# nanoporetech/isONclust2

Measured on AMD Instinct MI355X. Metric: reads/s clustered (sahlin mode, k=11 w=15), higher is better.
Workload: dtype u32

## Files before the change

### isonclust2_amd/csrc/ioc_align_gpu.hip

```cpp
#include <hip/hip_runtime.h>

#include <algorithm>
#include <chrono>
#include <cmath>
#include <cstdint>
#include <cstring>
#include <numeric>
#include <string>
#include <type_traits>
#include <vector>

#include "ioc_align_sink.h"
#include "ioc_internal.h"

namespace {

constexpr int ALN_C = 8;
constexpr int ALN_MAXW = 8;
constexpr int ALN_NEG = INT32_MIN / 4;
constexpr uint32_t ALN_LEN_SHIFT = 26;

struct AlnPairDev {
    uint32_t q_off, n;
    uint32_t r_off, m;
// ... 1539 lines not shown
    uint32_t* split;
    size_t resume_words;
};

int v2_tables(ioc_ctx* c, const V2Plan& pl, uint32_t help_wgs, V2Dev& t)
{
    hipStream_t s = c->stream;
    const uint32_t ncouples = pl.ncouples, np = pl.np;
    const size_t tab_bytes = size_t(ncouples) * sizeof(V2Couple) + size_t(np) * (sizeof(V2PairCk) + sizeof(V2PairEnd)) + size_t(pl.max_items) * sizeof(V2Item) + 256;
    IOC_TRY(ioc_reserve(c, c->a_cko, tab_bytes));
    uint8_t* tb = static_cast<uint8_t*>(c->a_cko.p);
    t.cps = reinterpret_cast<V2Couple*>(tb);
    t.pck = reinterpret_cast<V2PairCk*>(tb + size_t(ncouples) * sizeof(V2Couple));
    t.pend = reinterpret_cast<V2PairEnd*>(reinterpret_cast<uint8_t*>(t.pck) + size_t(np) * sizeof(V2PairCk));
    t.items = reinterpret_cast<V2Item*>(reinterpret_cast<uint8_t*>(t.pend) + size_t(np) * sizeof(V2PairEnd));
    IOC_CHK(c, hipMemcpyAsync(t.cps, pl.cps.data(), size_t(ncouples) * sizeof(V2Couple), hipMemcpyHostToDevice, s));
    IOC_CHK(c, hipMemcpyAsync(t.pck, pl.pck.data(), size_t(np) * sizeof(V2PairCk), hipMemcpyHostToDevice, s));
    IOC_CHK(c, hipMemcpyAsync(t.pend, pl.pend.data(), size_t(np) * sizeof(V2PairEnd), hipMemcpyHostToDevice, s));
    IOC_TRY(ioc_reserve(c, c->a_prof, size_t(pl.prof_total) * sizeof(uint4) + 256));
    IOC_TRY(ioc_reserve(c, c->a_ends2, size_t(np) * sizeof(int4)));
    IOC_TRY(ioc_reserve(c, c->a_lrow, (size_t(pl.lrow_total) + pl.best_total + 16) * sizeof(int2)));
    t.lrow = static_cast<int2*>(c->a_lrow.p);
    t.best = t.lrow + pl.lrow_total;
    t.ctl_words = ((16 + 2 * size_t(pl.max_flags) + np + 1) & ~size_t(1)) + 2;
    IOC_TRY(ioc_reserve(c, c->a_xflags, t.ctl_words * 4));
    t.ctl = static_cast<uint32_t*>(c->a_xflags.p);
    const size_t n_scratch = size_t(pl.max_pairs) + size_t(help_wgs) * V2_NHELP * V2_HBUF;
    t.resume_words = size_t(np) * V2_RESUME_WORDS + 2u * (size_t(pl.max_pairs) + 1u) + 4u + size_t(np) * V2_SPLIT_WORDS;
    IOC_TRY(ioc_reserve(c, c->a_bnd, n_scratch * sizeof(V2Scratch) + t.resume_words * 4));
    t.scratch = static_cast<V2Scratch*>(c->a_bnd.p);
    t.hscratch = t.scratch + pl.max_pairs;
    t.resume = reinterpret_cast<uint32_t*>(t.scratch + n_scratch);
    t.park = t.resume + size_t(np) * V2_RESUME_WORDS;
    t.early = t.park + size_t(pl.max_pairs) + 1u;
    t.gate = t.early + size_t(pl.max_pairs) + 1u;
    t.split = t.gate + 4u;
    return IOC_OK;
}

uint32_t v2_per_cu(const V2Plan& pl, size_t si, const V2Opts& o, bool few_couples)
{
    if (few_couples) return uint32_t(o.occ);
    uint64_t tiles = 0;
    uint32_t diags = 1;
    for (uint32_t k2 = pl.slices[si].first; k2 < pl.slices[si].first + pl.slices[si].second; ++k2) {
        const V2Couple& cp = pl.cps[k2];
        for (uint32_t b = 0; b < cp.nbands; ++b) tiles += uint32_t(cp.phi[b]) - uint32_t(cp.plo[b]) + 1u;
        diags = std::max(diags, cp.nbands + cp.nstrips - 1u);
    }
    const double x = double(tiles) / double(diags) / double(uint32_t(o.n_cu) * uint32_t(V2_WAVES));
    return x < 1.0 ? 1u : x < 2.75 ? std::min(2u, uint32_t(o.occ)) : uint32_t(o.occ);
}

int v2_slice(ioc_ctx* c, const V2Plan& pl, const V2Dev& t, size_t si, const V2Opts& o, const AlnParams& P, const uint32_t* d_order,
             int32_t* d_score, uint32_t* d_count, const hipEvent_t* ev, uint32_t* xe, const AlnOpsDev* od, StageTrace& tr)
{
    hipStream_t s = c->stream;
    const uint32_t k_first = pl.slices[si].first, n_couples = pl.slices[si].second;
    const uint32_t first_pair = 2u * k_first, n_pairs = std::min(pl.cnt, 2u * (k_first + n_couples)) - first_pair;
    const uint32_t n_items = pl.n_items[si], n_probe = pl.n_probe[si];
    const AlnPairDev* d_pairs = static_cast<const AlnPairDev*>(c->a_pairs.p);
    const uint8_t* d_pool = static_cast<const uint8_t*>(c->a_pool.p);
    uint32_t* d_ctl = t.ctl;
    const bool few_couples = n_couples <= o.few_limit;
    const uint32_t prog_every = few_couples ? 1u : 0u;
    const bool items_check = !pl.items.empty();
    if (items_check)
        IOC_CHK(c, hipMemsetAsync(t.items, 0xFF, size_t(n_items) * sizeof(V2Item), s));
    hipLaunchKernelGGL(k_fwd2_items, dim3(pl.n_diag[si], 2), dim3(V2_ITEMS_T), 0, s, t.cps, k_first, n_couples, n_probe, t.items, n_items);
    IOC_CHK(c, hipGetLastError());
    if (items_check) IOC_TRY(device_items_check(c, pl, t.items, si));
    hipLaunchKernelGGL(k_fwd2_prof, dim3(n_couples, pl.max_strips), dim3(128), 0, s, d_pairs, t.cps + k_first, d_pool, P, static_cast<uint4*>(c->a_prof.p));
    IOC_CHK(c, hipGetLastError());
    IOC_CHK(c, hipMemsetAsync(d_ctl, 0, t.ctl_words * 4, s));
    IOC_CHK(c, hipMemsetAsync(t.resume, 0, t.resume_words * 4, s));
    if (pl.tiles_skipped)
        IOC_CHK(c, hipMemsetAsync(t.lrow, 0x80, (size_t(pl.lrow_total) + pl.best_total) * sizeof(int2), s));
    if (getenv("IOC_ALIGN_V2_FAKE_TIMEOUT")) {
        const uint32_t one = 1;
        IOC_CHK(c, hipMemcpyAsync(d_ctl + 1, &one, 4, hipMemcpyHostToDevice, s));
    }
    IOC_CHK(c, hipEventRecord(ev[0], s));
    auto fwd = [&](decltype(&k_fwd2) kernel, uint32_t n_wg, const V2Item* items, uint32_t n) {
        hipLaunchKernelGGL(kernel, dim3(n_wg), dim3(64 * V2_WAVES), 0, s, d_pairs, t.cps, items, n, d_ctl, d_ctl + 16, d_ctl + 1, d_pool, P,
                           static_cast<uint32_t*>(c->a_ck.p), t.lrow, t.best, d_ctl + 16 + 2 * pl.max_flags, o.guard, static_cast<const uint4*>(c->a_prof.p),
                           reinterpret_cast<unsigned long long*>(d_ctl + t.ctl_words - 2), few_couples ? d_ctl + 16 + pl.max_flags : static_cast<uint32_t*>(nullptr),
                           prog_every);
    };
    if (n_probe) {
        fwd(k_fwd2, std::max(1u, std::min(uint32_t(o.occ) * uint32_t(o.n_cu), (n_probe + V2_WAVES - 1) / V2_WAVES)), t.items, n_probe);
        IOC_CHK(c, hipGetLastError());
        hipLaunchKernelGGL(k_fwd2_probe, dim3(n_couples), dim3(64), 0, s, d_pairs, t.cps + k_first, t.pend, static_cast<const uint32_t*>(c->a_ck.p), P);
        IOC_CHK(c, hipGetLastError());
        IOC_CHK(c, hipMemsetAsync(d_ctl, 0, 4, s));
    }
    tr.mark("v2_slice up to the probe");
    const uint32_t n_main = n_items - n_probe, per_cu = v2_per_cu(pl, si, o, few_couples);
    const uint32_t n_wg = std::max(1u, std::min(per_cu * uint32_t(o.n_cu), (n_main + V2_WAVES - 1) / V2_WAVES));
    const bool w2 = per_cu <= 2 && !getenv("IOC_ALIGN_V2_NO_W2");
    if (getenv("IOC_TRACE"))
        fprintf(stderr, "[ioc]   aligner v2: shape: slice %zu: %u couples, waits for %s, per_cu %u, n_wg %u, kernel %s, n_probe %u\n", si, n_couples,
                few_couples ? "rows" : "tiles", per_cu, n_wg, w2 ? "k_fwd2_w2" : "k_fwd2", n_probe);
    fwd(w2 ? k_fwd2_w2 : k_fwd2, n_wg, t.items + n_probe, n_main);
    IOC_CHK(c, hipGetLastError());
    const uint32_t n_help = std::min<uint32_t>(n_pairs, o.help_wgs);
    hipLaunchKernelGGL(k_fwd2_ends, dim3(n_pairs), dim3(64), 0, s, d_pairs, t.cps, d_order + first_pair, n_pairs, t.pend, t.lrow, t.best,
                       d_ctl + 16 + 2 * pl.max_flags, static_cast<int4*>(c->a_ends2.p), t.resume, t.early, o.side_help ? int(P.match) : 0, n_help);
    IOC_CHK(c, hipGetLastError());
    IOC_CHK(c, hipEventRecord(ev[1], s));
    auto help = [&](hipStream_t hs, uint32_t* list, uint32_t which, uint32_t* gate) {
        if (od)
            hipLaunchKernelGGL(k_trace2_help_ops, dim3(n_help), dim3(64 * V2_HWAVES), 0, hs, d_pairs, d_order + first_pair, d_pool, P,
                               static_cast<const uint32_t*>(c->a_ck.p), t.cps, t.pck, static_cast<const int4*>(c->a_ends2.p), t.scratch, t.hscratch,
                               t.resume, list, t.split, d_score, d_count, n_pairs, which, gate, *od);
        else
            hipLaunchKernelGGL(k_trace2_help, dim3(n_help), dim3(64 * V2_HWAVES), 0, hs, d_pairs, d_order + first_pair, d_pool, P,
                               static_cast<const uint32_t*>(c->a_ck.p), t.cps, t.pck, static_cast<const int4*>(c->a_ends2.p), t.scratch, t.hscratch,
                               t.resume, list, t.split, d_score, d_count, n_pairs, which, gate);
    };
    if (o.side_help) {
        IOC_CHK(c, hipEventRecord(c->ev_side[0], s));
        IOC_CHK(c, hipStreamWaitEvent(c->side_stream, c->ev_side[0], 0));
        help(c->side_stream, t.early, 2u, t.gate);
        IOC_CHK(c, hipGetLastError());
        IOC_CHK(c, hipEventRecord(c->ev_side[1], c->side_stream));
        hipLaunchKernelGGL(k_trace2_gate, dim3(1), dim3(1), 0, s, t.early, t.gate, n_help);
        IOC_CHK(c, hipGetLastError());
    }
    if (od)
        hipLaunchKernelGGL(k_trace2_ops, dim3((n_pairs + TR_WAVES - 1) / TR_WAVES), dim3(64 * TR_WAVES), 0, s, d_pairs, d_order + first_pair, d_pool, P,
                           static_cast<const uint32_t*>(c->a_ck.p), t.cps, t.pck, static_cast<const int4*>(c->a_ends2.p), t.scratch, t.resume, t.park,
                           t.split, d_score, d_count, n_pairs, o.deadline, o.deadline_cycles, *od);
    else
        hipLaunchKernelGGL(k_trace2, dim3((n_pairs + TR_WAVES - 1) / TR_WAVES), dim3(64 * TR_WAVES), 0, s, d_pairs, d_order + first_pair, d_pool, P,
                           static_cast<const uint32_t*>(c->a_ck.p), t.cps, t.pck, static_cast<const int4*>(c->a_ends2.p), t.scratch, t.resume, t.park,
                           t.split, d_score, d_count, n_pairs, o.deadline, o.deadline_cycles);
    IOC_CHK(c, hipGetLastError());
    if (o.side_help) IOC_CHK(c, hipStreamWaitEvent(s, c->ev_side[1], 0));
    if (o.deadline) {
        help(s, t.park, 1u, nullptr);
        IOC_CHK(c, hipGetLastError());
    }
    IOC_CHK(c, hipEventRecord(ev[2], s));
    unsigned long long cells_done = 0;
    IOC_CHK(c, hipMemcpyAsync(xe, d_ctl + 1, 4, hipMemcpyDeviceToHost, s));
    IOC_CHK(c, hipMemcpyAsync(&cells_done, d_ctl + t.ctl_words - 2, 8, hipMemcpyDeviceToHost, s));
    tr.mark("v2_slice other launches");
    IOC_CHK(c, hipStreamSynchronize(s));
    tr.mark("v2_slice wait (device)");
    c->tm.n_align_cells_computed += int64_t(cells_done);
    if (items_check) IOC_TRY(device_probe_report(c, pl, t.cps, si));
    return IOC_OK;
}

int v2_report(ioc_ctx* c, const std::vector<AlnPairDev>& dp, const uint32_t* order, const V2Plan& pl, const V2Dev& t, size_t si, uint32_t deadline)
{
    const bool rates = getenv("IOC_V2_TRACE_RATES") != nullptr, times = getenv("IOC_V2_TRACE_TIMES") != nullptr;
    if (!rates && !times) return IOC_OK;
    const uint32_t np = pl.np, first_pair = 2u * pl.slices[si].first;
    const uint32_t n_pairs = std::min(pl.cnt, 2u * (pl.slices[si].first + pl.slices[si].second)) - first_pair;
    std::vector<int4> he(np);
    IOC_CHK(c, hipMemcpy(he.data(), c->a_ends2.p, size_t(np) * sizeof(int4), hipMemcpyDeviceToHost));
    if (rates)
        for (uint32_t x = 0; x < n_pairs; ++x) {
            const uint32_t pid = order[first_pair + x];
            const AlnPairDev& d = dp[pid];
            fprintf(stderr, "[rate] e %.5f n %u m %u score %d per_base %.5f go %d flags %d corridor %u\n", double(d.e_sum), d.n, d.m, he[pid].x,
                    double(he[pid].x) / double(std::max(d.n, d.m)), d.gap_open, he[pid].w, pl.cps[pl.pend[pid].couple].corridor);
        }
    if (!times) return IOC_OK;
    std::vector<uint32_t> rw(size_t(np) * V2_RESUME_WORDS);
    IOC_CHK(c, hipMemcpy(rw.data(), t.resume, rw.size() * 4, hipMemcpyDeviceToHost));
    std::vector<uint32_t> ids(n_pairs);
// ... 139 lines not shown
    tr.mark("tile_counts");

    o.deadline = 4;
    if (const char* e = getenv("IOC_TRACE2_DEADLINE")) o.deadline = uint32_t(std::max(0, atoi(e)));
    if (const char* e = getenv("IOC_TRACE2_CYCLES")) o.deadline_cycles = (unsigned long long)std::max(0.0, atof(e));
    o.help_wgs = o.deadline ? std::min<uint32_t>(pl.max_pairs, uint32_t(o.n_cu)) : 0u;
    V2Dev t{};
    if ((r = v2_tables(c, pl, o.help_wgs, t)) != IOC_OK) return r;
    tr.mark("v2_tables");
    o.side_help = o.deadline && !(getenv("IOC_TRACE2_EARLY") && atoi(getenv("IOC_TRACE2_EARLY")) == 0);
    if (o.side_help && !c->side_stream) {
        IOC_CHK(c, hipStreamCreateWithFlags(&c->side_stream, hipStreamNonBlocking));
        for (auto& e : c->ev_side) IOC_CHK(c, hipEventCreateWithFlags(&e, hipEventDisableTiming));
    }
    EventSet evs;
    evs.v.assign(pl.slices.size() * 3, nullptr);
    for (auto& e : evs.v) IOC_CHK(c, hipEventCreate(&e));
    tr.mark("side stream, events");
    if (getenv("IOC_TRACE"))
        fprintf(stderr, "[ioc]   aligner v2: planning (couples, corridors, tile lists, tables) took the host %.3f ms\n",
                std::chrono::duration<double, std::milli>(std::chrono::steady_clock::now() - t_plan0).count());
    size_t evi = 0;
    bool bad = false;
    for (size_t si = 0; si < pl.slices.size() && !bad; ++si, evi += 3) {
        uint32_t xe = 0;
        if ((r = v2_slice(c, pl, t, si, o, P, d_order, d_score, d_count, &evs.v[evi], &xe, ops ? &ops->dev : nullptr, tr)) != IOC_OK) return r;
        if (ops && !xe) {
            const uint32_t x0 = 2u * pl.slices[si].first, x1 = std::min(cnt, 2u * (pl.slices[si].first + pl.slices[si].second));
            if ((r = ops_fetch(c, *ops, dp, order + x0, d_order + x0, x1 - x0, slice_ops[si])) != IOC_OK) return r;
        }
        if ((r = v2_report(c, dp, order, pl, t, si, o.deadline)) != IOC_OK) return r;
        bad = xe != 0;
    }
    add_elapsed(c, evs.v, evi);
    tr.mark("elapsed times");
    if (getenv("IOC_TRACE"))
        fprintf(stderr, "[ioc]   aligner v2: forward %.3f ms, traceback %.3f ms (device, all slices so far)%s\n", c->tm.ms_align_fwd,
                c->tm.ms_align_trace, bad ? " — a wait ran out: falling back to version 1" : "");
    *fell_back = bad;
    return IOC_OK;
}


enum class AlnRoute { normal, every_tile, v1_only };

struct AlnOut {
    int32_t* score;
    int64_t* windows;
    double* ratio;
    const AlnSink* ops = nullptr;
    void set(size_t i, int32_t s, int64_t w, double r) const
    {
        if (score) score[i] = s;
        if (windows) windows[i] = w;
        if (ratio) ratio[i] = r;
    }
};

// ... 620 lines not shown
```

### isonclust2_amd/csrc/ioc_align_v2.inc

```

constexpr int CK2 = 512;
constexpr int V2_WAVES = 4;
constexpr int V2_BLK_C = 8;
constexpr int V2_MAX_BANDS = 40;
static_assert(CK2 % TILE == 0 && CK2 == 64 * V2_BLK_C, "block geometry");

struct V2Couple {
    uint32_t pid[2];
    uint32_t nbands, nstrips;
    uint32_t tpb;
    uint32_t flag0;
    uint32_t mpad;
    uint32_t nq;
    uint64_t rdat;
    uint64_t rbase;
    uint64_t cdat;
    uint64_t cbase;
    uint64_t prof;
    uint32_t lrow0[2];
    uint32_t best0[2];
    uint16_t bstart[V2_MAX_BANDS + 1];
    uint16_t plo[V2_MAX_BANDS], phi[V2_MAX_BANDS];
    uint32_t corridor;
    uint16_t probe_band, probe_strip;
// ... 88 lines not shown
        e = umax2(e, h);
        h = umax2(T[c], e) - gd2;
        Hq[c] = h;
    }
    hql = h;
    el = e;
}

__device__ __forceinline__ uint32_t v2_par(uint32_t lds_byte_addr)
{
    uint32_t x;
    asm volatile("ds_read_b32 %0, %1\n\ts_waitcnt lgkmcnt(0)" : "=v"(x) : "v"(lds_byte_addr) : "memory");
    return x;
}

__device__ __forceinline__ void v2_lds_store(uint32_t lds_byte_addr, uint32_t v)
{
    asm volatile("ds_write_b32 %0, %1\n\ts_waitcnt lgkmcnt(0)" : : "v"(lds_byte_addr), "v"(v) : "memory");
}

enum V2Par : uint32_t {
    VP_N0 = 0, VP_N1, VP_M0, VP_M1, VP_GD0, VP_GD1, VP_LROW0, VP_LROW1, VP_BEST0, VP_BEST1, VP_PID0, VP_PID1,
    VP_RDAT_LO, VP_RDAT_HI, VP_RBASE_LO, VP_RBASE_HI, VP_CDAT_LO, VP_CDAT_HI, VP_CBASE_LO, VP_CBASE_HI,
    VP_MPAD, VP_NQ, VP_FLAG, VP_BAND, VP_STRIP, VP_COLIN_LO, VP_COLIN_HI, VP_RHI0, VP_RHI1, VP_COUNT = 32
};

__global__ void __launch_bounds__(128)
k_fwd2_prof(const AlnPairDev* __restrict__ pairs, const V2Couple* __restrict__ couples, const uint8_t* __restrict__ pool, AlnParams P, uint4* __restrict__ prof)
{
    const V2Couple& cp = couples[blockIdx.x];
    const uint32_t p = blockIdx.y;
    if (p >= cp.nstrips) return;
    const uint32_t h = threadIdx.x >> 6, lane = threadIdx.x & 63u;
    const bool have = cp.pid[h] != 0xFFFFFFFFu;
    const AlnPairDev pr = pairs[have ? cp.pid[h] : cp.pid[0]];
    const uint32_t m = have ? pr.m : 0u;
    const uint8_t* r = pool + pr.r_off;
    const int ge = P.gap_extend, gd = pr.gap_open - ge;
    const int cm = P.match + 2 * ge + gd, cx = P.mismatch + 2 * ge + gd;
    const uint32_t jb = p * (64u * FW_C) + lane * FW_C;
    uint32_t rpk[FW_C / 4];
#pragma unroll
    for (int c4 = 0; c4 < FW_C / 4; ++c4) {
        uint32_t w = 0;
#pragma unroll
        for (int e = 0; e < 4; ++e) w |= (have ? ref_byte(r, m, pr.rc, jb + c4 * 4 + e) : 0u) << (8 * e);
        rpk[c4] = w;
// ... 57 lines not shown
                cnt = min(dg, nb - 1u) - b_lo + 1u;
            }
        }
        s_scan[tid] = cnt;
        __syncthreads();
        for (uint32_t d = 1; d < V2_ITEMS_T; d <<= 1) {
            const uint32_t v = tid >= d ? s_scan[tid - d] : 0u;
            __syncthreads();
            s_scan[tid] += v;
            __syncthreads();
        }
        const uint32_t pos = running + s_scan[tid] - cnt;
        for (uint32_t i = 0; i < cnt; ++i)
            if (pos + i < n_items) items[pos + i] = V2Item{k_first + x, uint16_t(b_lo + i), uint16_t(dg - (b_lo + i))};
        running += s_scan[V2_ITEMS_T - 1];
        __syncthreads();
    }
}

static __device__ __forceinline__ void
v2_fwd_body(const AlnPairDev* __restrict__ pairs, const V2Couple* __restrict__ couples, const V2Item* __restrict__ items, uint32_t n_items,
       uint32_t* __restrict__ queue, uint32_t* __restrict__ flags, uint32_t* __restrict__ err, const uint8_t* __restrict__ pool, AlnParams P,
       uint32_t* __restrict__ arena, int2* __restrict__ lrow, int2* __restrict__ bandbest, uint32_t* __restrict__ ovf_out, int guard,
       const uint4* __restrict__ prof, unsigned long long* __restrict__ cells_done, uint32_t* __restrict__ prog, uint32_t prog_every)
{
    __shared__ __attribute__((aligned(16))) uint32_t s_look_all[V2_WAVES][3][128];
    __shared__ __attribute__((aligned(16))) uint32_t s_prof_all[V2_WAVES][2][5][64][4];
    __shared__ uint32_t s_par_all[V2_WAVES][VP_COUNT];
    const uint32_t lane = threadIdx.x & 63u;
    const uint32_t wv = uint32_t(__builtin_amdgcn_readfirstlane(int(threadIdx.x >> 6)));
    uint32_t(*s_look)[128] = s_look_all[wv];
    uint32_t* s_par = s_par_all[wv];
    const uint32_t par_addr = uint32_t(reinterpret_cast<uintptr_t>(s_par));
    auto par = [&](uint32_t k) -> uint32_t { return v2_par(par_addr + 4u * k); };
    auto par64 = [&](uint32_t k) -> uint64_t { return uint64_t(par(k)) | (uint64_t(par(k + 1u)) << 32); };
    constexpr uint32_t strip_cols = 64u * FW_C;
    const int ge = P.gap_extend;
    auto qcode = [](uint32_t ch) -> uint32_t {
        const uint32_t code = ch == 'A' ? 0u : ch == 'C' ? 1u : ch == 'G' ? 2u : ch == 'T' ? 3u : 4u;
        return code * 1024u;
    };
    uint32_t it = v2_dequeue(queue);
    while (it < n_items) {
        uint32_t band, p, r_lo, nblk[2];
        bool vh[2], last_band[2];
        bool left_ok = true;
        bool top_none = false;
        bool left_rows = false;
        uint32_t left_idx = 0, nblk_band = 0, left_avail = 0;
        const uint8_t* q[2];
        int base[2];
        uint32_t gd2;
        uint32_t Hp[FW_C], F[FW_C];
        uint32_t dg;
        uint64_t cb_off = 0;
        uint64_t co_off = 0;
        uint64_t rd_off = 0;
        uint64_t rb_off = 0;
        uint32_t mpad = 0, ncr = 0;
        {
            const V2Item item = items[it];
            const V2Couple cp = couples[item.couple];
            band = item.band;
            p = item.strip;
            if (p < cp.plo[band] || p > cp.phi[band] ||
                __builtin_amdgcn_readfirstlane(int(__hip_atomic_load(&flags[cp.flag0 + band * cp.nstrips + p], __ATOMIC_RELAXED, __HIP_MEMORY_SCOPE_AGENT))) != 0) {
                it = v2_dequeue(queue);
                continue;
            }
            const bool top_in = band > 0 && p >= cp.plo[band - 1u] && p <= cp.phi[band - 1u];
            const bool left_in = p > cp.plo[band];
            left_ok = p == 0 || left_in;
            top_none = band > 0 && !top_in;
            const bool corner_in = band > 0 && p > 0 && p - 1u >= cp.plo[band - 1u] && p - 1u <= cp.phi[band - 1u];
            if (top_in) (void)v2_wait(&flags[cp.flag0 + (band - 1u) * cp.nstrips + p], err);
            left_rows = prog != nullptr && left_in;
            left_idx = cp.flag0 + band * cp.nstrips + (p - 1u);
            {
                const uint32_t rows_b = min(max(cp.pid[0] != 0xFFFFFFFFu ? pairs[cp.pid[0]].n : 0u, cp.pid[1] != 0xFFFFFFFFu ? pairs[cp.pid[1]].n : 0u),
                                            uint32_t(cp.bstart[band + 1u]) * uint32_t(CK2));
                const uint32_t r0_b = uint32_t(cp.bstart[band]) * uint32_t(CK2);
                nblk_band = rows_b > r0_b ? (rows_b - r0_b + FW_R - 1) / FW_R : 0u;
            }
            if (left_in && !left_rows) (void)v2_wait(&flags[left_idx], err);
            if (left_rows) (void)v2_wait_rows(&prog[left_idx], &flags[left_idx], min(32u, nblk_band), err, left_avail);
            __builtin_amdgcn_fence(__ATOMIC_ACQUIRE, "agent");
            r_lo = uint32_t(cp.bstart[band]) * uint32_t(CK2);
            const uint32_t jb = p * strip_cols + lane * FW_C;
            uint32_t n[2], m[2], r_hi[2];
            int gd[2];
#pragma unroll
            for (int h = 0; h < 2; ++h) {
                const bool have = cp.pid[h] != 0xFFFFFFFFu;
                const AlnPairDev pr = pairs[have ? cp.pid[h] : cp.pid[0]];
                n[h] = have ? pr.n : 0u;
                m[h] = have ? pr.m : 0u;
                q[h] = pool + pr.q_off;
                gd[h] = pr.gap_open - ge;
                r_hi[h] = min(n[h], uint32_t(cp.bstart[band + 1u]) * uint32_t(CK2));
                nblk[h] = r_hi[h] > r_lo ? (r_hi[h] - r_lo + FW_R - 1) / FW_R : 0u;
                const uint32_t nstr = (m[h] + strip_cols - 1) / strip_cols;
                vh[h] = have && p < nstr && nblk[h] > 0;
                last_band[h] = vh[h] && r_hi[h] == n[h];
            }
            gd2 = packu(uint32_t(gd[0]), uint32_t(gd[1]));
            mpad = cp.mpad;
            rd_off = cp.rdat + jb;
            rb_off = cp.rbase + uint64_t(jb / 16u) * 2u;
            {
                uint32_t nmx = max(n[0], n[1]);
                ncr = nmx ? (nmx - 1u) / uint32_t(CK2) : 0u;
            }
            {
                const uint64_t e0 = uint64_t((jb + FW_C) / CK2 - ((jb + FW_C) >= uint32_t(CK2) ? 1u : 0u)) * cp.nq + r_lo / 4u;
                co_off = cp.cdat + e0 * 8u;
                cb_off = cp.cbase + e0 * 2u;
            }
            const uint64_t colin = p ? uint64_t(p * (strip_cols / CK2) - 1u) * cp.nq : 0;
            __builtin_amdgcn_fence(__ATOMIC_RELEASE, "workgroup");
            __builtin_amdgcn_wave_barrier();
            if (lane == 0) {
                s_par[VP_N0] = n[0];
                s_par[VP_N1] = n[1];
                s_par[VP_M0] = m[0];
                s_par[VP_M1] = m[1];
                s_par[VP_GD0] = uint32_t(gd[0]);
                s_par[VP_GD1] = uint32_t(gd[1]);
                s_par[VP_LROW0] = cp.lrow0[0];
                s_par[VP_LROW1] = cp.lrow0[1];
                s_par[VP_BEST0] = cp.best0[0];
                s_par[VP_BEST1] = cp.best0[1];
                s_par[VP_PID0] = cp.pid[0];
                s_par[VP_PID1] = cp.pid[1];
                s_par[VP_RDAT_LO] = uint32_t(cp.rdat);
                s_par[VP_RDAT_HI] = uint32_t(cp.rdat >> 32);
                s_par[VP_RBASE_LO] = uint32_t(cp.rbase);
                s_par[VP_RBASE_HI] = uint32_t(cp.rbase >> 32);
                s_par[VP_CDAT_LO] = uint32_t(cp.cdat);
                s_par[VP_CDAT_HI] = uint32_t(cp.cdat >> 32);
                s_par[VP_CBASE_LO] = uint32_t(cp.cbase);
                s_par[VP_CBASE_HI] = uint32_t(cp.cbase >> 32);
                s_par[VP_MPAD] = cp.mpad;
                s_par[VP_NQ] = cp.nq;
                s_par[VP_FLAG] = cp.flag0 + band * cp.nstrips + p;
                s_par[VP_BAND] = band;
                s_par[VP_STRIP] = p;
                s_par[VP_COLIN_LO] = uint32_t(colin);
                s_par[VP_COLIN_HI] = uint32_t(colin >> 32);
                s_par[VP_RHI0] = r_hi[0];
                s_par[VP_RHI1] = r_hi[1];
            }
            int Ha[2][FW_C], Fa[2][FW_C], dga[2];
#pragma unroll
            for (int h = 0; h < 2; ++h) {
                if (!vh[h]) {
#pragma unroll
                    for (int c = 0; c < FW_C; ++c) Ha[h][c] = Fa[h][c] = 0;
                    dga[h] = 0;
                } else if (r_lo > 0 && !top_in) {
#pragma unroll
                    for (int c = 0; c < FW_C; ++c) Ha[h][c] = Fa[h][c] = ALN_NEG;
                    dga[h] = ALN_NEG;
                } else if (r_lo == 0) {
                    const int b0 = ge * int(jb) - gd[h];
#pragma unroll
                    for (int c = 0; c < FW_C; ++c) {
                        Ha[h][c] = b0 + ge * (c + 1);
                        Fa[h][c] = ALN_NEG;
                    }
                    dga[h] = b0;
                } else {
                    const uint32_t ckr = r_lo / CK2 - 1u;
                    const uint32_t* rh = arena + cp.rdat + uint64_t(2u * ckr) * cp.mpad;
// ... 24 lines not shown
                    base[h] = v2_half(d[0], h) + (h ? bb.y : bb.x) - U16_BIAS;
                } else
                base[h] = __builtin_amdgcn_readfirstlane(Ha[h][0]) - U16_BIAS;
            }
#pragma unroll
            for (int c = 0; c < FW_C; ++c) {
                const bool in0 = vh[0] && jb + c < m[0], in1 = vh[1] && jb + c < m[1];
                Hp[c] = packu(in0 ? clampu16(Ha[0][c] - base[0]) : uint32_t(U16_BIAS), in1 ? clampu16(Ha[1][c] - base[1]) : uint32_t(U16_BIAS));
                F[c] = packu(in0 ? clampu16(Fa[0][c] - base[0]) : uint32_t(U16_BIAS), in1 ? clampu16(Fa[1][c] - base[1]) : uint32_t(U16_BIAS));
            }
            dg = packu(clampu16(dga[0] - base[0]), clampu16(dga[1] - base[1]));
            {
                const uint4* pp = prof + cp.prof + uint64_t(p) * (2u * 5u * 64u) + lane;
#pragma unroll
                for (int h = 0; h < 2; ++h)
#pragma unroll
                    for (int code = 0; code < 5; ++code) {
                        const uint4 w = pp[(uint32_t(h) * 5u + uint32_t(code)) * 64u];
                        *reinterpret_cast<uint4*>(&s_prof_all[wv][h][code][lane][0]) = w;
                    }
            }
        }
        const uint32_t jb = p * strip_cols + lane * FW_C;
        const uint32_t nsteps = max(nblk[0], nblk[1]) + 63u;
        uint32_t lanef = 0;
        int lastc[2];
        uint32_t ncl[2];
        bool strip_has_lastc = false;
        __builtin_amdgcn_fence(__ATOMIC_RELEASE, "workgroup");
        __builtin_amdgcn_wave_barrier();
        __builtin_amdgcn_fence(__ATOMIC_ACQUIRE, "workgroup");
        {
            const uint32_t jr = jb + FW_C;
            bool any_right = false;
#pragma unroll
            for (int h = 0; h < 2; ++h) {
                const uint32_t mh = par(VP_M0 + h);
                const bool hc = vh[h] && jb < mh;
                ncl[h] = vh[h] ? min(64u, (mh - p * strip_cols + FW_C - 1) / FW_C) : 0u;
                lastc[h] = (vh[h] && mh - 1 >= jb && mh - 1 < jb + FW_C) ? int(mh - 1 - jb) : -1;
                strip_has_lastc = strip_has_lastc || (vh[h] && uint64_t(p + 1u) * strip_cols >= mh);
                any_right = any_right || (vh[h] && jr < mh);
                lanef |= (hc ? 1u : 0u) << h;
                lanef |= (lastc[h] >= 0 ? 4u : 0u) << h;
            }
            if ((jr % CK2) == 0 && any_right) lanef |= 16u;
        }
// ... 35 lines not shown
                en[h] = left_edge(h, row);
            }
            qn = qq[0] | (qq[1] << 16);
        };
        fetch(0);
        publish(0);
        fetch(1);
        __builtin_amdgcn_fence(__ATOMIC_RELEASE, "workgroup");
        __builtin_amdgcn_wave_barrier();
        __builtin_amdgcn_fence(__ATOMIC_ACQUIRE, "workgroup");
        uint4 nxh, nxe, nxq;
        nxh = *reinterpret_cast<const uint4*>(&s_look[0][0]);
        nxe = *reinterpret_cast<const uint4*>(&s_look[1][0]);
        nxq = *reinterpret_cast<const uint4*>(&s_look[2][0]);
        {
            const uint32_t q4[FW_R] = {nxq.x, nxq.y, nxq.z, nxq.w};
#pragma unroll
            for (int rr = 0; rr < FW_R; ++rr) qc[rr] = from_left_or(qc[rr], q4[rr]);
        }
        int bc[2] = {ALN_NEG, ALN_NEG};
        uint32_t bc_i[2] = {0, 0};
        uint32_t ovf = 0;

        auto step = [&](const uint32_t s, auto first) __attribute__((always_inline)) {
            if (decltype(first)::value && (s & (64 / FW_R - 1)) == 0) {
                if (s) {
                    int dl[2];
#pragma unroll
                    for (int h = 0; h < 2; ++h) {
                        const uint32_t lr = s + 1u > nblk[h] ? min(63u, s + 1u - nblk[h]) : 0u;
                        const int ref = __builtin_amdgcn_readlane(int(Hp[0]), int(lr));
                        dl[h] = max(v2_half(uint32_t(ref), h) - U16_BIAS, 0);
                        if (!vh[h] || lr >= ncl[h]) dl[h] = 0;
                        base[h] += dl[h];
                    }
                    const uint32_t d2 = packu(uint32_t(dl[0]), uint32_t(dl[1]));
                    {
                        uint32_t mx = Hp[0], mn = Hp[0];
#pragma unroll
                        for (int c = 1; c < FW_C; ++c) {
                            mx = umax2(mx, Hp[c]);
                            mn = umin2(mn, Hp[c]);
                        }
                        const int bi = int(s) - int(lane);
#pragma unroll
                        for (int h = 0; h < 2; ++h) {
                            const int hi_v = v2_half(mx, h) - U16_BIAS, lo_v = v2_half(mn, h) - U16_BIAS;
                            if ((lanef >> h & 1u) && bi >= (top_none ? 1 : 0) && uint32_t(bi) < nblk[h] && (hi_v > guard || lo_v < -guard)) {
// ... 6 lines not shown
                    }
#pragma unroll
                    for (int c = 0; c < FW_C; ++c) {
                        Hp[c] = usubs2(Hp[c], d2);
                        F[c] = usubs2(F[c], d2);
                    }
                    dg = usubs2(dg, d2);
#pragma unroll
                    for (int rr = 0; rr < FW_R; ++rr) {
                        hl[rr] = usubs2(hl[rr], d2);
                        el[rr] = usubs2(el[rr], d2);
                    }
                    nxh = uint4{usubs2(nxh.x, d2), usubs2(nxh.y, d2), usubs2(nxh.z, d2), usubs2(nxh.w, d2)};
                    nxe = uint4{usubs2(nxe.x, d2), usubs2(nxe.y, d2), usubs2(nxe.z, d2), usubs2(nxe.w, d2)};
                    const uint32_t cur = ((s / (64 / FW_R)) & 1u) * 64u + lane;
                    s_look[0][cur] = usubs2(s_look[0][cur], d2);
                    s_look[1][cur] = usubs2(s_look[1][cur], d2);
                }
                const uint32_t blk = s / (64 / FW_R) + 1u;
                if (prog != nullptr && s >= 64u && (prog_every <= 1u || (s / 16u) % prog_every == 0u)) {
                    asm volatile("s_waitcnt vmcnt(0)" ::: "memory");
                    __builtin_amdgcn_fence(__ATOMIC_RELEASE, "agent");
                    asm volatile("s_waitcnt vmcnt(0)" ::: "memory");
                    __hip_atomic_store(&prog[uint32_t(__builtin_amdgcn_readfirstlane(int(par(VP_FLAG))))], s - 63u, __ATOMIC_RELAXED, __HIP_MEMORY_SCOPE_AGENT);
                }
                publish(blk);
                if (left_rows) {
                    const uint32_t need_rows = min(16u * (blk + 2u), nblk_band);
                    if (need_rows > left_avail) {
                        (void)v2_wait_rows(&prog[left_idx], &flags[left_idx], need_rows, err, left_avail);
                        __builtin_amdgcn_fence(__ATOMIC_ACQUIRE, "agent");
                    }
                }
                fetch(blk + 1u);
            }
            {
                const uint32_t h4[FW_R] = {nxh.x, nxh.y, nxh.z, nxh.w}, e4[FW_R] = {nxe.x, nxe.y, nxe.z, nxe.w};
#pragma unroll
                for (int rr = 0; rr < FW_R; ++rr) {
                    hl[rr] = from_left_or(hl[rr], h4[rr]);
                    el[rr] = from_left_or(el[rr], e4[rr]);
                }
                const uint32_t nx = ((s + 1u) * FW_R) & 127u;
                nxh = *reinterpret_cast<const uint4*>(&s_look[0][nx]);
                nxe = *reinterpret_cast<const uint4*>(&s_look[1][nx]);
                nxq = *reinterpret_cast<const uint4*>(&s_look[2][nx]);
            }
// ... 1 lines not shown
            bool act[2];
#pragma unroll
            for (int h = 0; h < 2; ++h) act[h] = (lanef >> h & 1u) && bi >= 0 && uint32_t(bi) < nblk[h];
            if (act[0] || act[1]) {
                const bool special = strip_has_lastc || (last_band[0] && s + 1u >= nblk[0] && s + 1u - nblk[0] < 64u) ||
                                     (last_band[1] && s + 1u >= nblk[1] && s + 1u - nblk[1] < 64u);
                auto row_cells = [&](int rr) __attribute__((always_inline)) {
                    const uint32_t hl_in = hl[rr];
                    const uint4 xa = *reinterpret_cast<const uint4*>(profA + (qc[rr] & 0xFFFFu));
                    const uint4 xb = *reinterpret_cast<const uint4*>(profB + (qc[rr] >> 16));
                    cells_u16(Hp, F, xa, xb, hl[rr], el[rr], dg, gd2);
                    dg = hl_in;
                };
#pragma unroll
                for (int rr = 0; rr < FW_R; ++rr) {
                    row_cells(rr);
                    if (special) {

#pragma unroll
                        for (int h = 0; h < 2; ++h) {
                            const uint32_t i = r_lo + uint32_t(bi) * FW_R + rr;
                            const uint32_t nh = par(VP_N0 + h), mh = par(VP_M0 + h);
                            const int gdh = int(par(VP_GD0 + h));
                            if (act[h] && i < nh) {
                                if (lastc[h] >= 0) {
                                    const uint32_t lc = uint32_t(lastc[h]);
                                    const bool b0 = lc & 1u, b1 = lc & 2u, b2 = lc & 4u, b3 = lc & 8u;
                                    const uint32_t s0 = b0 ? Hp[1] : Hp[0], s1 = b0 ? Hp[3] : Hp[2], s2 = b0 ? Hp[5] : Hp[4], s3 = b0 ? Hp[7] : Hp[6],
                                                   s4 = b0 ? Hp[9] : Hp[8], s5 = b0 ? Hp[11] : Hp[10], s6 = b0 ? Hp[13] : Hp[12], s7 = b0 ? Hp[15] : Hp[14];
                                    const uint32_t u0 = b1 ? s1 : s0, u1 = b1 ? s3 : s2, u2 = b1 ? s5 : s4, u3 = b1 ? s7 : s6;
                                    const uint32_t v0 = b2 ? u1 : u0, v1 = b2 ? u3 : u2;
                                    int hm = v2_half(b3 ? v1 : v0, h) + base[h];
                                    hm += gdh - ge * int(i + 1u + mh);
                                    if (hm > bc[h]) {
                                        bc[h] = hm;
                                        bc_i[h] = i + 1u;
                                    }
                                }
                                if (i + 1u == nh) {
                                    int br = ALN_NEG;
                                    uint32_t bj = 0;
                                    const int b0 = base[h] + gdh - ge * int(nh + jb);
#pragma unroll
                                    for (int c = 0; c < FW_C; ++c) {
                                        const int ht = v2_half(Hp[c], h) + b0 - ge * (c + 1);
                                        if (jb + c < mh && ht > br) {
// ... 25 lines not shown
#pragma unroll
                        for (int c = 0; c < FW_C; c += 4) {
                            oh[c / 4] = uint4{Hp[c], Hp[c + 1], Hp[c + 2], Hp[c + 3]};
                            of[c / 4] = uint4{F[c], F[c + 1], F[c + 2], F[c + 3]};
                        }
                        reinterpret_cast<int2*>(arena + rb_off)[uint64_t(ckr1 - 1u) * (mpad / 16u)] = int2{base[0], base[1]};
                    }
                }
            }
            {
                const uint32_t q4[FW_R] = {nxq.x, nxq.y, nxq.z, nxq.w};
#pragma unroll
                for (int rr = 0; rr < FW_R; ++rr) qc[rr] = from_left_or(qc[rr], q4[rr]);
            }
        };
        {
            uint32_t s = 0;
            for (; s + 1u < nsteps; s += 2) {
                step(s, std::true_type{});
                step(s + 1u, std::false_type{});
            }
            for (; s < nsteps; ++s) step(s, std::true_type{});
        }
#pragma unroll
        for (int h = 0; h < 2; ++h) {
            if (lastc[h] >= 0) bandbest[par(VP_BEST0 + h) + band] = int2{bc[h], int(bc_i[h])};
            if ((ovf >> h) & 1u) {
                const uint32_t pidh = par(VP_PID0 + h);
                if (pidh != 0xFFFFFFFFu) atomicOr(&ovf_out[pidh], 1u);
            }
        }
        if (lane == 0) {
            unsigned long long cells = 0;
#pragma unroll
            for (int h = 0; h < 2; ++h)
                if (vh[h]) cells += (unsigned long long)(par(VP_RHI0 + h) - r_lo) * (unsigned long long)min(strip_cols, par(VP_M0 + h) - p * strip_cols);
            atomicAdd(cells_done, cells);
        }
        const uint32_t my_flag = uint32_t(__builtin_amdgcn_readfirstlane(int(par(VP_FLAG))));
        asm volatile("s_waitcnt vmcnt(0)" ::: "memory");
        __builtin_amdgcn_fence(__ATOMIC_RELEASE, "agent");
        asm volatile("s_waitcnt vmcnt(0)" ::: "memory");
        __hip_atomic_store(&flags[my_flag], 1u, __ATOMIC_RELAXED, __HIP_MEMORY_SCOPE_AGENT);
        it = v2_dequeue(queue);
    }
}

#define V2_FWD_ARGS                                                                                                                        \
    const AlnPairDev *__restrict__ pairs, const V2Couple *__restrict__ couples, const V2Item *__restrict__ items, uint32_t n_items,        \
        uint32_t *__restrict__ queue, uint32_t *__restrict__ flags, uint32_t *__restrict__ err, const uint8_t *__restrict__ pool, AlnParams P, \
        uint32_t *__restrict__ arena, int2 *__restrict__ lrow, int2 *__restrict__ bandbest, uint32_t *__restrict__ ovf_out, int guard,     \
        const uint4 *__restrict__ prof, unsigned long long *__restrict__ cells_done, uint32_t *__restrict__ prog, uint32_t prog_every
__global__ void __launch_bounds__(64 * V2_WAVES) __attribute__((amdgpu_waves_per_eu(3, 8))) k_fwd2(V2_FWD_ARGS)
{
    v2_fwd_body(pairs, couples, items, n_items, queue, flags, err, pool, P, arena, lrow, bandbest, ovf_out, guard, prof, cells_done, prog, prog_every);
}
__global__ void __launch_bounds__(64 * V2_WAVES) __attribute__((amdgpu_waves_per_eu(2, 2))) k_fwd2_w2(V2_FWD_ARGS)
{
    v2_fwd_body(pairs, couples, items, n_items, queue, flags, err, pool, P, arena, lrow, bandbest, ovf_out, guard, prof, cells_done, prog, prog_every);
}


struct V2PairEnd {
    uint32_t lrow0, best0, nbands, couple;
    int32_t cert;
};
constexpr uint32_t V2_RESUME_WORDS = 16;
constexpr uint32_t V2_SPLIT_WORDS = 24;

__global__ void __launch_bounds__(64)
k_fwd2_probe(const AlnPairDev* __restrict__ pairs, V2Couple* __restrict__ couples, V2PairEnd* __restrict__ pe, const uint32_t* __restrict__ arena, AlnParams P)
{
    V2Couple& cp = couples[blockIdx.x];
    if (!cp.corridor) return;
    const uint32_t lane = threadIdx.x;
    const uint32_t strip_cols = 64u * FW_C;
    const uint32_t R = uint32_t(cp.bstart[cp.probe_band + 1u]) * uint32_t(CK2);
    const uint32_t ckr = R / uint32_t(CK2) - 1u;
    const uint32_t* rh = arena + cp.rdat + uint64_t(2u * ckr) * cp.mpad;
    const int2* rb = reinterpret_cast<const int2*>(arena + cp.rbase) + uint64_t(ckr) * (cp.mpad / 16u);
    bool wrong = false;
    uint32_t nmax = 0, mmax = 0, need = 0, need_raw = 0;
// ... 957 lines not shown
```

Baseline: 65090.

## Chain wavefront tiles into the next band without leaving the kernel loop

When a tile nears the end of its band, the wave can claim the tile directly below in the same strip and keep streaming rows into it, instead of finishing and dequeuing a new item. The previous tile's flag and band-best are published once the wavefront has passed the boundary. A claims array stops other waves from processing a tile that has already been linked. The goal is to cut the dependency stalls and pipeline fill/drain at band boundaries, at the cost of extra atomics, more complex bookkeeping and a larger control buffer. This path is enabled by default.

```diff
diff --git a/isonclust2_amd/csrc/ioc_align_gpu.hip b/isonclust2_amd/csrc/ioc_align_gpu.hip
--- a/isonclust2_amd/csrc/ioc_align_gpu.hip
+++ b/isonclust2_amd/csrc/ioc_align_gpu.hip
@@ -1585,7 +1585,7 @@
     IOC_TRY(ioc_reserve(c, c->a_lrow, (size_t(pl.lrow_total) + pl.best_total + 16) * sizeof(int2)));
     t.lrow = static_cast<int2*>(c->a_lrow.p);
     t.best = t.lrow + pl.lrow_total;
-    t.ctl_words = ((16 + 2 * size_t(pl.max_flags) + np + 1) & ~size_t(1)) + 2;
+    t.ctl_words = ((16 + 3 * size_t(pl.max_flags) + np + 1) & ~size_t(1)) + 2;
     IOC_TRY(ioc_reserve(c, c->a_xflags, t.ctl_words * 4));
     t.ctl = static_cast<uint32_t*>(c->a_xflags.p);
     const size_t n_scratch = size_t(pl.max_pairs) + size_t(help_wgs) * V2_NHELP * V2_HBUF;
@@ -1616,7 +1616,7 @@
 }
 
 int v2_slice(ioc_ctx* c, const V2Plan& pl, const V2Dev& t, size_t si, const V2Opts& o, const AlnParams& P, const uint32_t* d_order,
-             int32_t* d_score, uint32_t* d_count, const hipEvent_t* ev, uint32_t* xe, const AlnOpsDev* od, StageTrace& tr)
+             int32_t* d_score, uint32_t* d_count, const hipEvent_t* ev, uint32_t* xe, uint32_t* link_sum, const AlnOpsDev* od, StageTrace& tr)
 {
     hipStream_t s = c->stream;
     const uint32_t k_first = pl.slices[si].first, n_couples = pl.slices[si].second;
@@ -1627,6 +1627,8 @@
     uint32_t* d_ctl = t.ctl;
     const bool few_couples = n_couples <= o.few_limit;
     const uint32_t prog_every = few_couples ? 1u : 0u;
+    const bool links = !(getenv("IOC_ALIGN_V2_LINK") && atoi(getenv("IOC_ALIGN_V2_LINK")) == 0);
+    uint32_t* const d_claims = links ? d_ctl + 16 + 2 * pl.max_flags + pl.np : static_cast<uint32_t*>(nullptr);
     const bool items_check = !pl.items.empty();
     if (items_check)
         IOC_CHK(c, hipMemsetAsync(t.items, 0xFF, size_t(n_items) * sizeof(V2Item), s));
@@ -1644,14 +1646,14 @@
         IOC_CHK(c, hipMemcpyAsync(d_ctl + 1, &one, 4, hipMemcpyHostToDevice, s));
     }
     IOC_CHK(c, hipEventRecord(ev[0], s));
-    auto fwd = [&](decltype(&k_fwd2) kernel, uint32_t n_wg, const V2Item* items, uint32_t n) {
+    auto fwd = [&](decltype(&k_fwd2) kernel, uint32_t n_wg, const V2Item* items, uint32_t n, uint32_t link_mode) {
         hipLaunchKernelGGL(kernel, dim3(n_wg), dim3(64 * V2_WAVES), 0, s, d_pairs, t.cps, items, n, d_ctl, d_ctl + 16, d_ctl + 1, d_pool, P,
                            static_cast<uint32_t*>(c->a_ck.p), t.lrow, t.best, d_ctl + 16 + 2 * pl.max_flags, o.guard, static_cast<const uint4*>(c->a_prof.p),
                            reinterpret_cast<unsigned long long*>(d_ctl + t.ctl_words - 2), few_couples ? d_ctl + 16 + pl.max_flags : static_cast<uint32_t*>(nullptr),
-                           prog_every);
+                           prog_every, d_claims, link_mode);
     };
     if (n_probe) {
-        fwd(k_fwd2, std::max(1u, std::min(uint32_t(o.occ) * uint32_t(o.n_cu), (n_probe + V2_WAVES - 1) / V2_WAVES)), t.items, n_probe);
+        fwd(k_fwd2, std::max(1u, std::min(uint32_t(o.occ) * uint32_t(o.n_cu), (n_probe + V2_WAVES - 1) / V2_WAVES)), t.items, n_probe, 2u);
         IOC_CHK(c, hipGetLastError());
         hipLaunchKernelGGL(k_fwd2_probe, dim3(n_couples), dim3(64), 0, s, d_pairs, t.cps + k_first, t.pend, static_cast<const uint32_t*>(c->a_ck.p), P);
         IOC_CHK(c, hipGetLastError());
@@ -1664,7 +1666,7 @@
     if (getenv("IOC_TRACE"))
         fprintf(stderr, "[ioc]   aligner v2: shape: slice %zu: %u couples, waits for %s, per_cu %u, n_wg %u, kernel %s, n_probe %u\n", si, n_couples,
                 few_couples ? "rows" : "tiles", per_cu, n_wg, w2 ? "k_fwd2_w2" : "k_fwd2", n_probe);
-    fwd(w2 ? k_fwd2_w2 : k_fwd2, n_wg, t.items + n_probe, n_main);
+    fwd(w2 ? k_fwd2_w2 : k_fwd2, n_wg, t.items + n_probe, n_main, 1u);
     IOC_CHK(c, hipGetLastError());
     const uint32_t n_help = std::min<uint32_t>(n_pairs, o.help_wgs);
     hipLaunchKernelGGL(k_fwd2_ends, dim3(n_pairs), dim3(64), 0, s, d_pairs, t.cps, d_order + first_pair, n_pairs, t.pend, t.lrow, t.best,
@@ -1708,10 +1710,13 @@
     unsigned long long cells_done = 0;
     IOC_CHK(c, hipMemcpyAsync(xe, d_ctl + 1, 4, hipMemcpyDeviceToHost, s));
     IOC_CHK(c, hipMemcpyAsync(&cells_done, d_ctl + t.ctl_words - 2, 8, hipMemcpyDeviceToHost, s));
+    uint32_t link_counts[3] = {0, 0, 0};
+    if (getenv("IOC_TRACE")) IOC_CHK(c, hipMemcpyAsync(link_counts, d_ctl + 4, sizeof link_counts, hipMemcpyDeviceToHost, s));
     tr.mark("v2_slice other launches");
     IOC_CHK(c, hipStreamSynchronize(s));
     tr.mark("v2_slice wait (device)");
     c->tm.n_align_cells_computed += int64_t(cells_done);
+    for (int x = 0; x < 3; ++x) link_sum[x] += link_counts[x];
     if (items_check) IOC_TRY(device_probe_report(c, pl, t.cps, si));
     return IOC_OK;
 }
@@ -1897,9 +1902,10 @@
                 std::chrono::duration<double, std::milli>(std::chrono::steady_clock::now() - t_plan0).count());
     size_t evi = 0;
     bool bad = false;
+    uint32_t link_sum[3] = {0, 0, 0};
     for (size_t si = 0; si < pl.slices.size() && !bad; ++si, evi += 3) {
         uint32_t xe = 0;
-        if ((r = v2_slice(c, pl, t, si, o, P, d_order, d_score, d_count, &evs.v[evi], &xe, ops ? &ops->dev : nullptr, tr)) != IOC_OK) return r;
+        if ((r = v2_slice(c, pl, t, si, o, P, d_order, d_score, d_count, &evs.v[evi], &xe, link_sum, ops ? &ops->dev : nullptr, tr)) != IOC_OK) return r;
         if (ops && !xe) {
             const uint32_t x0 = 2u * pl.slices[si].first, x1 = std::min(cnt, 2u * (pl.slices[si].first + pl.slices[si].second));
             if ((r = ops_fetch(c, *ops, dp, order + x0, d_order + x0, x1 - x0, slice_ops[si])) != IOC_OK) return r;
@@ -1909,6 +1915,9 @@
     }
     add_elapsed(c, evs.v, evi);
     tr.mark("elapsed times");
+    if (getenv("IOC_TRACE"))
+        fprintf(stderr, "[ioc]   aligner v2: links: %u of %u (%u without a left side, %u with the left tile done)\n", link_sum[1] + link_sum[2], link_sum[0],
+                link_sum[1], link_sum[2]);
     if (getenv("IOC_TRACE"))
         fprintf(stderr, "[ioc]   aligner v2: forward %.3f ms, traceback %.3f ms (device, all slices so far)%s\n", c->tm.ms_align_fwd,
                 c->tm.ms_align_trace, bad ? " — a wait ran out: falling back to version 1" : "");
diff --git a/isonclust2_amd/csrc/ioc_align_v2.inc b/isonclust2_amd/csrc/ioc_align_v2.inc
--- a/isonclust2_amd/csrc/ioc_align_v2.inc
+++ b/isonclust2_amd/csrc/ioc_align_v2.inc
@@ -134,7 +134,9 @@
 enum V2Par : uint32_t {
     VP_N0 = 0, VP_N1, VP_M0, VP_M1, VP_GD0, VP_GD1, VP_LROW0, VP_LROW1, VP_BEST0, VP_BEST1, VP_PID0, VP_PID1,
     VP_RDAT_LO, VP_RDAT_HI, VP_RBASE_LO, VP_RBASE_HI, VP_CDAT_LO, VP_CDAT_HI, VP_CBASE_LO, VP_CBASE_HI,
-    VP_MPAD, VP_NQ, VP_FLAG, VP_BAND, VP_STRIP, VP_COLIN_LO, VP_COLIN_HI, VP_RHI0, VP_RHI1, VP_COUNT = 32
+    VP_MPAD, VP_NQ, VP_FLAG, VP_BAND, VP_STRIP, VP_COLIN_LO, VP_COLIN_HI, VP_RHI0, VP_RHI1,
+    VP_COUPLE, VP_FLAG_PREV, VP_BND_PREV,
+    VP_COUNT = 32
 };
 
 __global__ void __launch_bounds__(128)
@@ -238,8 +240,11 @@
 v2_fwd_body(const AlnPairDev* __restrict__ pairs, const V2Couple* __restrict__ couples, const V2Item* __restrict__ items, uint32_t n_items,
        uint32_t* __restrict__ queue, uint32_t* __restrict__ flags, uint32_t* __restrict__ err, const uint8_t* __restrict__ pool, AlnParams P,
        uint32_t* __restrict__ arena, int2* __restrict__ lrow, int2* __restrict__ bandbest, uint32_t* __restrict__ ovf_out, int guard,
-       const uint4* __restrict__ prof, unsigned long long* __restrict__ cells_done, uint32_t* __restrict__ prog, uint32_t prog_every)
-{
+       const uint4* __restrict__ prof, unsigned long long* __restrict__ cells_done, uint32_t* __restrict__ prog, uint32_t prog_every,
+       uint32_t* __restrict__ claims, uint32_t link_mode)
+{
+    uint32_t* const link_stats = queue + 4;
+    constexpr uint32_t NEVER = 0xFFFFFFFFu;
     __shared__ __attribute__((aligned(16))) uint32_t s_look_all[V2_WAVES][3][128];
     __shared__ __attribute__((aligned(16))) uint32_t s_prof_all[V2_WAVES][2][5][64][4];
     __shared__ uint32_t s_par_all[V2_WAVES][VP_COUNT];
@@ -264,6 +269,8 @@
         bool top_none = false;
         bool left_rows = false;
         uint32_t left_idx = 0, nblk_band = 0, left_avail = 0;
+        uint32_t bnd = 0;
+        uint32_t link_at = NEVER;
         const uint8_t* q[2];
         int base[2];
         uint32_t gd2;
@@ -280,7 +287,9 @@
             band = item.band;
             p = item.strip;
             if (p < cp.plo[band] || p > cp.phi[band] ||
-                __builtin_amdgcn_readfirstlane(int(__hip_atomic_load(&flags[cp.flag0 + band * cp.nstrips + p], __ATOMIC_RELAXED, __HIP_MEMORY_SCOPE_AGENT))) != 0) {
+                __builtin_amdgcn_readfirstlane(int(__hip_atomic_load(&flags[cp.flag0 + band * cp.nstrips + p], __ATOMIC_RELAXED, __HIP_MEMORY_SCOPE_AGENT))) != 0 ||
+                (claims != nullptr &&
+                 __builtin_amdgcn_readfirstlane(int(__hip_atomic_load(&claims[cp.flag0 + band * cp.nstrips + p], __ATOMIC_RELAXED, __HIP_MEMORY_SCOPE_AGENT))) != 0)) {
                 it = v2_dequeue(queue);
                 continue;
             }
@@ -300,6 +309,10 @@
             }
             if (left_in && !left_rows) (void)v2_wait(&flags[left_idx], err);
             if (left_rows) (void)v2_wait_rows(&prog[left_idx], &flags[left_idx], min(32u, nblk_band), err, left_avail);
+            if (claims != nullptr && v2_dequeue(&claims[left_idx + 1u]) != 0u) {
+                it = v2_dequeue(queue);
+                continue;
+            }
             __builtin_amdgcn_fence(__ATOMIC_ACQUIRE, "agent");
             r_lo = uint32_t(cp.bstart[band]) * uint32_t(CK2);
             const uint32_t jb = p * strip_cols + lane * FW_C;
@@ -320,6 +333,9 @@
                 last_band[h] = vh[h] && r_hi[h] == n[h];
             }
             gd2 = packu(uint32_t(gd[0]), uint32_t(gd[1]));
+            if (claims != nullptr && band + 1u < cp.nbands && nblk_band >= 128u &&
+                max(vh[0] ? n[0] : 0u, vh[1] ? n[1] : 0u) > uint32_t(cp.bstart[band + 1u]) * uint32_t(CK2))
+                link_at = nblk_band - 32u;
             mpad = cp.mpad;
             rd_off = cp.rdat + jb;
             rb_off = cp.rbase + uint64_t(jb / 16u) * 2u;
@@ -365,6 +381,9 @@
                 s_par[VP_COLIN_HI] = uint32_t(colin >> 32);
                 s_par[VP_RHI0] = r_hi[0];
                 s_par[VP_RHI1] = r_hi[1];
+                s_par[VP_COUPLE] = item.couple;
+                s_par[VP_FLAG_PREV] = 0;
+                s_par[VP_BND_PREV] = 0;
             }
             int Ha[2][FW_C], Fa[2][FW_C], dga[2];
 #pragma unroll
@@ -435,7 +454,7 @@
             }
         }
         const uint32_t jb = p * strip_cols + lane * FW_C;
-        const uint32_t nsteps = max(nblk[0], nblk[1]) + 63u;
+        uint32_t nsteps = max(nblk[0], nblk[1]) + 63u;
         uint32_t lanef = 0;
         int lastc[2];
         uint32_t ncl[2];
@@ -517,8 +536,87 @@
         uint32_t bc_i[2] = {0, 0};
         uint32_t ovf = 0;
 
+        auto finish_prev = [&]() {
+            const uint32_t bp = uint32_t(__builtin_amdgcn_readfirstlane(int(par(VP_BND_PREV))));
+#pragma unroll
+            for (int h = 0; h < 2; ++h)
+                if (lastc[h] >= 0 && nblk[h] <= bnd && nblk[h] > bp) bandbest[par(VP_BEST0 + h) + band - 1u] = int2{bc[h], int(bc_i[h])};
+            const uint32_t prev_flag = uint32_t(__builtin_amdgcn_readfirstlane(int(par(VP_FLAG_PREV))));
+            asm volatile("s_waitcnt vmcnt(0)" ::: "memory");
+            __builtin_amdgcn_fence(__ATOMIC_RELEASE, "agent");
+            asm volatile("s_waitcnt vmcnt(0)" ::: "memory");
+            __hip_atomic_store(&flags[prev_flag], 1u, __ATOMIC_RELAXED, __HIP_MEMORY_SCOPE_AGENT);
+            uint32_t keep = 0xFFFFFFFFu, fill = 0u;
+#pragma unroll
+            for (int h = 0; h < 2; ++h)
+                if (!vh[h] || nblk[h] <= bnd) {
+                    keep &= ~(0xFFFFu << (16 * h));
+                    fill |= uint32_t(U16_BIAS) << (16 * h);
+                }
+            if (keep != 0xFFFFFFFFu) {
+#pragma unroll
+                for (int c = 0; c < FW_C; ++c) {
+                    Hp[c] = (Hp[c] & keep) | fill;
+                    F[c] = (F[c] & keep) | fill;
+                }
+#pragma unroll
+                for (int rr = 0; rr < FW_R; ++rr) {
+                    hl[rr] = (hl[rr] & keep) | fill;
+                    el[rr] &= keep;
+                }
+                dg = (dg & keep) | fill;
+            }
+        };
+        auto link_decide = [&]() {
+            const V2Couple* cq = couples + uint32_t(__builtin_amdgcn_readfirstlane(int(par(VP_COUPLE))));
+            const uint32_t nb = band + 1u;
+            const uint32_t lo = cq->plo[nb], hi = cq->phi[nb];
+            const uint32_t fi = cq->flag0 + nb * cq->nstrips + p;
+            bool go = p >= lo && p <= hi;
+            if (link_mode == 2u) go = go && nb <= uint32_t(cq->probe_band) && p <= uint32_t(cq->probe_strip);
+            uint32_t kind = 0;
+            if (go) {
+                if (p == 0u || p == lo) kind = 1u;
+                else if (__builtin_amdgcn_readfirstlane(int(__hip_atomic_load(&flags[fi - 1u], __ATOMIC_RELAXED, __HIP_MEMORY_SCOPE_AGENT))) != 0) kind = 2u;
+                go = kind != 0u && __builtin_amdgcn_readfirstlane(int(__hip_atomic_load(&flags[fi], __ATOMIC_RELAXED, __HIP_MEMORY_SCOPE_AGENT))) == 0 &&
+                     v2_dequeue(&claims[fi]) == 0u;
+            }
+            link_at = NEVER;
+            if (!go) return;
+            __builtin_amdgcn_fence(__ATOMIC_ACQUIRE, "agent");
+            const uint32_t bend = uint32_t(cq->bstart[nb + 1u]) * uint32_t(CK2);
+            uint32_t nn[2], rh[2];
+#pragma unroll
+            for (int h = 0; h < 2; ++h) {
+                nn[h] = uint32_t(__builtin_amdgcn_readfirstlane(int(par(VP_N0 + h))));
+                rh[h] = min(nn[h], bend);
+                if (vh[h]) {
+                    nblk[h] = (rh[h] - r_lo + FW_R - 1) / FW_R;
+                    last_band[h] = rh[h] == nn[h];
+                }
+            }
+            const uint32_t old_flag = par(VP_FLAG);
+            v2_lds_store(par_addr + 4u * VP_FLAG_PREV, old_flag);
+            v2_lds_store(par_addr + 4u * VP_BND_PREV, bnd);
+            v2_lds_store(par_addr + 4u * VP_FLAG, fi);
+            v2_lds_store(par_addr + 4u * VP_BAND, nb);
+            v2_lds_store(par_addr + 4u * VP_RHI0, rh[0]);
+            v2_lds_store(par_addr + 4u * VP_RHI1, rh[1]);
+            bnd = nblk_band;
+            nblk_band = (min(max(nn[0], nn[1]), bend) - r_lo + FW_R - 1) / FW_R;
+            nsteps = max(nblk[0], nblk[1]) + 63u;
+            band = nb;
+            left_ok = p == 0u || p > lo;
+            left_rows = false;
+            if (nb + 1u < cq->nbands && max(vh[0] ? nn[0] : 0u, vh[1] ? nn[1] : 0u) > bend) link_at = nblk_band - 32u;
+            (void)v2_dequeue(link_stats);
+            (void)v2_dequeue(link_stats + kind);
+        };
+
         auto step = [&](const uint32_t s, auto first) __attribute__((always_inline)) {
             if (decltype(first)::value && (s & (64 / FW_R - 1)) == 0) {
+                if (s == link_at) link_decide();
+                if (bnd != 0u && s == bnd + 64u) finish_prev();
                 if (s) {
                     int dl[2];
 #pragma unroll
@@ -571,7 +669,11 @@
                     asm volatile("s_waitcnt vmcnt(0)" ::: "memory");
                     __builtin_amdgcn_fence(__ATOMIC_RELEASE, "agent");
                     asm volatile("s_waitcnt vmcnt(0)" ::: "memory");
-                    __hip_atomic_store(&prog[uint32_t(__builtin_amdgcn_readfirstlane(int(par(VP_FLAG))))], s - 63u, __ATOMIC_RELAXED, __HIP_MEMORY_SCOPE_AGENT);
+                    if (s >= bnd + 64u)
+                        __hip_atomic_store(&prog[uint32_t(__builtin_amdgcn_readfirstlane(int(par(VP_FLAG))))], s - 63u - bnd, __ATOMIC_RELAXED, __HIP_MEMORY_SCOPE_AGENT);
+                    else
+                        __hip_atomic_store(&prog[uint32_t(__builtin_amdgcn_readfirstlane(int(par(VP_FLAG_PREV))))],
+                                           s - 63u - uint32_t(__builtin_amdgcn_readfirstlane(int(par(VP_BND_PREV)))), __ATOMIC_RELAXED, __HIP_MEMORY_SCOPE_AGENT);
                 }
                 publish(blk);
                 if (left_rows) {
@@ -619,6 +721,11 @@
                             const uint32_t i = r_lo + uint32_t(bi) * FW_R + rr;
                             const uint32_t nh = par(VP_N0 + h), mh = par(VP_M0 + h);
                             const int gdh = int(par(VP_GD0 + h));
+                            if (rr == 0 && bnd != 0u && uint32_t(bi) == bnd && act[h] && lastc[h] >= 0) {
+                                bandbest[par(VP_BEST0 + h) + band - 1u] = int2{bc[h], int(bc_i[h])};
+                                bc[h] = ALN_NEG;
+                                bc_i[h] = 0;
+                            }
                             if (act[h] && i < nh) {
                                 if (lastc[h] >= 0) {
                                     const uint32_t lc = uint32_t(lastc[h]);
@@ -690,9 +797,10 @@
             }
             for (; s < nsteps; ++s) step(s, std::true_type{});
         }
+        if (bnd != 0u && nsteps <= bnd + 64u) finish_prev();
 #pragma unroll
         for (int h = 0; h < 2; ++h) {
-            if (lastc[h] >= 0) bandbest[par(VP_BEST0 + h) + band] = int2{bc[h], int(bc_i[h])};
+            if (lastc[h] >= 0 && (bnd == 0u || nblk[h] > bnd)) bandbest[par(VP_BEST0 + h) + band] = int2{bc[h], int(bc_i[h])};
             if ((ovf >> h) & 1u) {
                 const uint32_t pidh = par(VP_PID0 + h);
                 if (pidh != 0xFFFFFFFFu) atomicOr(&ovf_out[pidh], 1u);
@@ -704,6 +812,7 @@
             for (int h = 0; h < 2; ++h)
                 if (vh[h]) cells += (unsigned long long)(par(VP_RHI0 + h) - r_lo) * (unsigned long long)min(strip_cols, par(VP_M0 + h) - p * strip_cols);
             atomicAdd(cells_done, cells);
+            atomicAdd(link_stats, 1u);
         }
         const uint32_t my_flag = uint32_t(__builtin_amdgcn_readfirstlane(int(par(VP_FLAG))));
         asm volatile("s_waitcnt vmcnt(0)" ::: "memory");
@@ -718,14 +827,17 @@
     const AlnPairDev *__restrict__ pairs, const V2Couple *__restrict__ couples, const V2Item *__restrict__ items, uint32_t n_items,        \
         uint32_t *__restrict__ queue, uint32_t *__restrict__ flags, uint32_t *__restrict__ err, const uint8_t *__restrict__ pool, AlnParams P, \
         uint32_t *__restrict__ arena, int2 *__restrict__ lrow, int2 *__restrict__ bandbest, uint32_t *__restrict__ ovf_out, int guard,     \
-        const uint4 *__restrict__ prof, unsigned long long *__restrict__ cells_done, uint32_t *__restrict__ prog, uint32_t prog_every
+        const uint4 *__restrict__ prof, unsigned long long *__restrict__ cells_done, uint32_t *__restrict__ prog, uint32_t prog_every,  \
+        uint32_t *__restrict__ claims, uint32_t link_mode
 __global__ void __launch_bounds__(64 * V2_WAVES) __attribute__((amdgpu_waves_per_eu(3, 8))) k_fwd2(V2_FWD_ARGS)
 {
-    v2_fwd_body(pairs, couples, items, n_items, queue, flags, err, pool, P, arena, lrow, bandbest, ovf_out, guard, prof, cells_done, prog, prog_every);
+    v2_fwd_body(pairs, couples, items, n_items, queue, flags, err, pool, P, arena, lrow, bandbest, ovf_out, guard, prof, cells_done, prog, prog_every, claims,
+                link_mode);
 }
 __global__ void __launch_bounds__(64 * V2_WAVES) __attribute__((amdgpu_waves_per_eu(2, 2))) k_fwd2_w2(V2_FWD_ARGS)
 {
-    v2_fwd_body(pairs, couples, items, n_items, queue, flags, err, pool, P, arena, lrow, bandbest, ovf_out, guard, prof, cells_done, prog, prog_every);
+    v2_fwd_body(pairs, couples, items, n_items, queue, flags, err, pool, P, arena, lrow, bandbest, ovf_out, guard, prof, cells_done, prog, prog_every, claims,
+                link_mode);
 }
 
 
```

After: 67120, median of 6. 1.03x the previous value.
